# yuxng/PoseCNN

Measured on AMD Instinct MI355X. Metric: RGB-D frames/sec (640x480, 21 classes), higher is better.
Workload: dtype f32

## Files before the change

### posecnn_amd/_lib.py

```python
import ctypes
import os
from ctypes import (POINTER, c_char_p, c_float, c_int, c_int32, c_int64, c_size_t, c_uint64, c_void_p)

_HERE = os.path.dirname(os.path.abspath(__file__))
LIB_PATH = os.path.join(_HERE, "libposecnn_hip.so")

PCNN_OK = 0
PCNN_EINVAL = -1
PCNN_EWORKSPACE = -2
PCNN_EHIP = -3
PCNN_ENULL = -4

MAX_ROI = 128
HOUGH_ROWS_CAPACITY = MAX_ROI * 9
VERTEX_CHANNELS = 3
POSE_CHANNELS = 4

_P = c_void_p

SIGNATURES = {
    "pcnn_abi_version": (c_int, []),
    "pcnn_last_error_string": (c_char_p, []),
    "pcnn_status_string": (c_char_p, [c_int]),
    "pcnn_hough_voting_workspace_bytes": (c_int, [c_int, c_int, c_int, c_int, c_float, c_int, c_int, POINTER(c_size_t)]),
# ... 129 lines not shown
    "pcnn_bias_relu_train_bwd": (c_int, [_P, _P, c_int64, c_int, c_int, _P, _P, _P, c_size_t, _P]),
}

POSE3D_SIGNATURES = {
    "pcnn_pose3d_workspace_bytes": (c_int, [c_int, c_int, c_int, c_int, c_int, POINTER(c_size_t)]),
    "pcnn_pose3d_prepare_fwd": (c_int, [_P, _P, _P, _P, _P, c_float, c_int, c_int, c_int, c_int, _P, _P, _P, _P]),
    "pcnn_pose3d_sample_fwd": (c_int, [_P, _P, _P, _P, _P, _P, c_uint64, c_uint64, c_int, c_int, c_int, c_int, c_int, c_int, c_int,
                                       c_float, c_float, _P, _P, _P, _P, _P]),
    "pcnn_pose3d_round_fwd": (c_int, [_P, _P, _P, _P, _P, c_int, c_int, c_int, c_int, c_int, c_int, c_int, c_int, c_float,
                                      _P, _P, _P, _P]),
    "pcnn_pose3d_estimate_fwd": (c_int, [_P, _P, _P, _P, _P, _P, c_float, c_uint64, c_uint64, c_int, c_int, c_int, c_int,
                                         c_int, c_int, c_int, c_int, c_int, c_float, c_float, c_int,
                                         _P, _P, _P, _P, _P, _P, c_size_t, _P]),
}


def profile_enable(on=True):
    check("pcnn_profile_enable", lib().pcnn_profile_enable(1 if on else 0))


def profile_report(reset=True):
    import json
    L = lib()
    n = L.pcnn_profile_report(None, 0)
    buf = ctypes.create_string_buffer(int(n) + 16)
    L.pcnn_profile_report(buf, len(buf))
    if reset:
        L.pcnn_profile_reset()
    rep = json.loads(buf.value.decode())
    return {k.strip("()"): v for k, v in rep.items()}
# ... 8 lines not shown
        self.status = status


def lib():
    global _lib
    if _lib is None:
        if not os.path.exists(LIB_PATH):
            raise RuntimeError(
                "libposecnn_hip.so not found at %s — build it with "
                "`python -c 'import __graft_entry__ as g; g.build()'` or "
                "`make -C posecnn_amd/csrc`. There is no CPU/PyTorch fallback." % LIB_PATH)
        import torch
        handle = ctypes.CDLL(LIB_PATH)
        for name, (res, args) in list(SIGNATURES.items()) + list(TRAIN_SIGNATURES.items()) + list(FRONTEND_SIGNATURES.items()) +\
                list(SYNTH_SIGNATURES.items()) + list(AUGMENT_SIGNATURES.items()) + list(LOSS_SIGNATURES.items()) +\
                list(VERTEX_LOSS_SIGNATURES.items()) + list(TRUNK_TRAIN_SIGNATURES.items()) + list(POSE3D_SIGNATURES.items()):
            fn = getattr(handle, name)
            fn.restype = res
            fn.argtypes = args
        if handle.pcnn_abi_version() != 2:
            raise RuntimeError("libposecnn_hip.so ABI version mismatch")
        _lib = handle
    return _lib


def check(fn_name, status):
    if status != PCNN_OK:
        msg = lib().pcnn_last_error_string()
        msg = msg.decode("utf-8", "replace") if msg else ""
        if status in (PCNN_EINVAL, PCNN_ENULL):
            raise ValueError("%s: %s" % (fn_name, msg))
# ... 2 lines not shown
```

### posecnn_amd/csrc/mfma_ring.h

```cpp
#pragma once

namespace pcnn {

typedef float v4f __attribute__((ext_vector_type(4)));

__device__ __forceinline__ void glds16_s(const char* sbase, unsigned voff, unsigned lds_addr)
{
  asm volatile("s_mov_b32 m0, %2\n\tglobal_load_lds_dwordx4 %0, %1"
               :: "v"(voff), "s"(sbase), "s"(lds_addr) : "memory", "m0");
}

__device__ __forceinline__ int ring_src_col(int lr, int row) { return (lr ^ (row & 15)) * 4; }
__device__ __forceinline__ unsigned ring_chunk_bytes(int j, int lk, int lr) { return (unsigned)(((4 * j + lk) ^ lr) * 16); }

}

#define RING_DSREAD_B128(DST, ADDR, OFF) asm volatile("ds_read_b128 %0, %1 offset:%2" : "=v"(DST) : "v"(ADDR), "i"(OFF))
```

### posecnn_amd/csrc/wino_mfma.hip

```cpp
#include <cstdlib>

#include "pcnn_device.h"
#include "mfma_ring.h"

namespace {

using namespace pcnn;

constexpr int WM_BC = 64;
constexpr int WM_KC = 64;
constexpr int WM_LD = 64;
constexpr int WM_NBUF = 3;
constexpr int WM_BT = 32;
constexpr int WM_NW = 4;
constexpr int WM_UB = WM_BC / 4 / WM_NW;

enum : int {
  ABL_NO_BARRIER = 1,
  ABL_NO_DMA = 2,
  ABL_NO_LDS_READS = 4,
  ABL_NO_MFMA = 8,
  ABL_NO_FOLD = 16,
  ABL_NO_EPILOGUE = 32,
  ABL_L2_OPERANDS = 64,
  ABL_NO_STORES = 128,
  ABL_EPI_REGS_ONLY = 256,
  ABL_NT_STORES = 512,
};

template <int POOL, int ABL = 0>
__global__ __launch_bounds__(64 * WM_NW, 2) void wino43_mfma_kernel(
    const float* __restrict__ v, const float* __restrict__ ut, const float* __restrict__ bias,
    float* __restrict__ y, float* __restrict__ ypool, int H, int W, int Cin, int Cout, int Ht, int Wt,
    long long T, long long tiles_per_group, int relu, int nbt, int ncb, int ksplit, long long ysplit_stride, int mode)
{
  constexpr int RING = WM_NBUF * (WM_BT + 64) * WM_LD, STAGE2 = 2 * WM_BT * 4 * 64;
  __shared__ __attribute__((aligned(16))) float smem[RING > STAGE2 ? RING : STAGE2];

  const int x = blockIdx.x & 7, q = blockIdx.x >> 3;
  const bool cbmajor = (mode & 1) != 0;
  const int cb = cbmajor ? x : q % ncb;
  const int tb = cbmajor ? q : (q / ncb) * 8 + x;
  if (tb >= nbt) return;
  const int tb_data = (ABL & ABL_L2_OPERANDS) ? 0 : tb, cb_data = (ABL & ABL_L2_OPERANDS) ? 0 : cb;
  y += (long long)blockIdx.y * ysplit_stride;

  const int tid = threadIdx.x, lane = tid & 63;
  const int wave = __builtin_amdgcn_readfirstlane(tid >> 6);
  const int lr = lane & 15, lk = lane >> 4;
  const int nbg = (int)((tiles_per_group + WM_BT - 1) / WM_BT);
  const int grp = tb / nbg;
// ... 32 lines not shown
#pragma unroll
  for (int b = 0; b < 2; b++)
#pragma unroll
    for (int i = 0; i < 2; i++)
#pragma unroll
      for (int o = 0; o < 16; o++) yo2[b][i][o] = (v2f){0.f, 0.f};

#define WM_DMA(BUF, VO, UO)                                                  \
  if constexpr (!(ABL & ABL_NO_DMA)) {                                       \
    const char* vs_ = vbase + (VO) * 4;                                      \
    const char* us_ = ubase + (UO) * 4;                                      \
    const unsigned la_ = lds_a0 + (unsigned)(BUF) * (WM_BT * WM_LD * 4);       \
    const unsigned lb_ = lds_b0 + (unsigned)(BUF) * (64 * WM_LD * 4);          \
    glds16_s(vs_, va0, la_);                                                 \
    glds16_s(vs_, va1, la_ + 4 * WM_LD * 4);                                 \
    _Pragma("unroll") for (int i_ = 0; i_ < WM_UB; i_++)                      \
      glds16_s(us_, ub[i_], lb_ + 4 * i_ * WM_LD * 4);                        \
  }

  int pnu = 0, pxi = 0, pkc = 0;
  long long pvo = (long long)ks * NK * WM_KC, puo = pvo;
  const long long kback = (long long)(NK - 1) * WM_KC;
  const long long dvx = 6 * vplane - kback, dux = 6 * uplane - kback;
  const long long dvn = -29 * vplane - kback, dun = -29 * uplane - kback;
#define WM_PF_ADVANCE()                                                                          \
  do {                                                                                           \
    if (pkc + 1 < NK) { pkc++; pvo += WM_KC; puo += WM_KC; }                    \
    else if (pxi < 5) { pkc = 0; pxi++; pvo += dvx; puo += dux; }        \
    else if (pnu < 5) { pkc = 0; pxi = 0; pnu++; pvo += dvn; puo += dun; }        \
  } while (0)
  { WM_DMA(0, pvo, puo); WM_PF_ADVANCE(); }
  { WM_DMA(1, pvo, puo); WM_PF_ADVANCE(); }
  int cur = 0;

  const int ra0 = lr * WM_LD, rb = (16 * wave + lr) * WM_LD;

  v4f xa0[2], xa1[2], xb[2], ya0[2], ya1[2], yb[2];
  const unsigned lds0 = (unsigned)(unsigned long long)(__attribute__((address_space(3))) float*)smem;
  unsigned adA[4], adB[4];
#pragma unroll
  for (int j = 0; j < 4; j++) {
    const unsigned chb = ring_chunk_bytes(j, lk, lr);
    adA[j] = lds0 + (unsigned)ra0 * 4u + chb;
    adB[j] = lds0 + (unsigned)(WM_NBUF * WM_BT * WM_LD + rb) * 4u + chb;
  }
#define WM_DSREAD(DST, ADDR, OFF)                                                                     \
  if constexpr (!(ABL & ABL_NO_LDS_READS)) RING_DSREAD_B128(DST, ADDR, OFF);                          \
  else asm volatile("" : "+v"(DST) : "v"(ADDR))
#define WM_READ_AT(SA0, SA1, SB, G0, CUR)                                                             \
  _Pragma("unroll") for (int g_ = 0; g_ < 2; g_++) {                                                  \
    WM_DSREAD(SB[g_], adB[(G0) + g_], (CUR) * (64 * WM_LD * 4));                                      \
    WM_DSREAD(SA0[g_], adA[(G0) + g_], (CUR) * (WM_BT * WM_LD * 4));                                  \
    WM_DSREAD(SA1[g_], adA[(G0) + g_], (CUR) * (WM_BT * WM_LD * 4) + 4096);       \
  }
#define WM_READ(SA0, SA1, SB, G0)                                                                     \
  if constexpr (ABL & ABL_NO_LDS_READS) { WM_READ_AT(SA0, SA1, SB, G0, 0); }    \
  else if (cur == 0) { WM_READ_AT(SA0, SA1, SB, G0, 0); }                                             \
  else if (cur == 1) { WM_READ_AT(SA0, SA1, SB, G0, 1); }                                             \
  else { WM_READ_AT(SA0, SA1, SB, G0, 2); }
  static_assert(WM_NBUF == 3, "WM_READ dispatches over a ring of three buffers");
#define WM_MFMA1(SA0, SA1, SB, G, ACC)                                                                \
  if constexpr (ABL & ABL_NO_MFMA) { asm volatile("" :: "v"(SA0[G]), "v"(SA1[G]), "v"(SB[G])); } else \
  _Pragma("unroll") for (int i_ = 0; i_ < 4; i_++) {                                                  \
    ACC[0] = __builtin_amdgcn_mfma_f32_16x16x4f32(SA0[G][i_], SB[G][i_], ACC[0], 0, 0, 0);            \
    ACC[1] = __builtin_amdgcn_mfma_f32_16x16x4f32(SA1[G][i_], SB[G][i_], ACC[1], 0, 0, 0);            \
  }
#define WM_MFMA(SA0, SA1, SB, ACC)                                                                    \
  WM_MFMA1(SA0, SA1, SB, 0, ACC) WM_MFMA1(SA0, SA1, SB, 1, ACC)
#define WM_MFMA1_Z(SA0, SA1, SB, G, ACC)                                                              \
  if constexpr (ABL & ABL_NO_MFMA) { asm volatile("" :: "v"(SA0[G]), "v"(SA1[G]), "v"(SB[G])); } else { \
    const v4f z_ = (v4f){0.f, 0.f, 0.f, 0.f};                                                         \
    ACC[0] = __builtin_amdgcn_mfma_f32_16x16x4f32(SA0[G][0], SB[G][0], z_, 0, 0, 0);                  \
    ACC[1] = __builtin_amdgcn_mfma_f32_16x16x4f32(SA1[G][0], SB[G][0], z_, 0, 0, 0);                  \
    _Pragma("unroll") for (int i_ = 1; i_ < 4; i_++) {                                                \
// ... 19 lines not shown
        _Pragma("unroll") for (int x_ = 0; x_ < 6; x_++) m_[x_] = (v2f){acc[x_][b_][2 * h_], acc[x_][b_][2 * h_ + 1]}; \
        const v2f s_ = m_[1] + m_[2], d_ = m_[1] - m_[2], S_ = m_[3] + m_[4], D_ = m_[3] - m_[4];   \
        t_[0] = (m_[0] + s_) + S_;                                                                  \
        t_[1] = __builtin_elementwise_fma((v2f){2.f, 2.f}, D_, d_);                                 \
        t_[2] = __builtin_elementwise_fma((v2f){4.f, 4.f}, S_, s_);                                 \
        t_[3] = __builtin_elementwise_fma((v2f){8.f, 8.f}, D_, d_) + m_[5];                         \
        _Pragma("unroll") for (int a_ = 0; a_ < 4; a_++) {                                          \
          yo2[b_][h_][4 * a_ + 0] = __builtin_elementwise_fma(t_[a_], (v2f){c0, c0}, yo2[b_][h_][4 * a_ + 0]); \
          yo2[b_][h_][4 * a_ + 1] = __builtin_elementwise_fma(t_[a_], (v2f){c1, c1}, yo2[b_][h_][4 * a_ + 1]); \
          yo2[b_][h_][4 * a_ + 2] = __builtin_elementwise_fma(t_[a_], (v2f){c2, c2}, yo2[b_][h_][4 * a_ + 2]); \
          yo2[b_][h_][4 * a_ + 3] = __builtin_elementwise_fma(t_[a_], (v2f){c3, c3}, yo2[b_][h_][4 * a_ + 3]); \
        }                                                                                           \
      }                                                                                             \
  }

#define WM_STAGE(XI, XP)                                                                              \
  do {                                                                                                \
    if constexpr (ABL & ABL_NO_BARRIER) asm volatile("s_waitcnt vmcnt(4) lgkmcnt(0)" ::: "memory");   \
    else asm volatile("s_waitcnt vmcnt(6) lgkmcnt(0)\n\ts_barrier" ::: "memory");                     \
    WM_READ(xa0, xa1, xb, 0);                                                                         \
    __builtin_amdgcn_sched_barrier(0);    \
    if (kc > 0) { WM_MFMA(ya0, ya1, yb, acc[XI]); }                                                   \
    else if ((XI) > 0) { WM_MFMA(ya0, ya1, yb, acc[XP]); }                                            \
    else if (nu > 0) { WM_MFMA(ya0, ya1, yb, acc[5]); WM_FOLD(nup); }                                 \
    {                                                                                                 \
      const int nb = cur >= 1 ? cur - 1 : 2;            \
      WM_DMA(nb, pvo, puo);                                                                           \
      WM_PF_ADVANCE();                                                                                \
    }                                                                                                 \
    __builtin_amdgcn_sched_barrier(0);                                                                \
    asm volatile("s_waitcnt lgkmcnt(0)" ::: "memory");           \
    __builtin_amdgcn_sched_barrier(0);                                                                \
    if (kc == 0) { WM_MFMA1_Z(xa0, xa1, xb, 0, acc[XI]); }           \
    else { WM_MFMA1(xa0, xa1, xb, 0, acc[XI]); }                                                      \
    __builtin_amdgcn_sched_barrier(0);    \
    WM_READ(ya0, ya1, yb, 2);                                                                         \
    __builtin_amdgcn_sched_barrier(0);                                                                \
    WM_MFMA1(xa0, xa1, xb, 1, acc[XI]);                                                               \
    __builtin_amdgcn_sched_barrier(0);                                                                \
    asm volatile("s_waitcnt lgkmcnt(0)" ::: "memory");    \
    cur = cur == 2 ? 0 : cur + 1;                                                                     \
  } while (0)
  static_assert(2 + WM_UB == 6, "the stage barrier's vmcnt(6) counts the 2 + WM_UB DMA instructions a wave issues per stage");

  int nup = -1;
  for (int nu = 0; nu < 6; nu++) {
    for (int kc = 0; kc < NK; kc++) WM_STAGE(0, 5);
    for (int kc = 0; kc < NK; kc++) WM_STAGE(1, 0);
    for (int kc = 0; kc < NK; kc++) WM_STAGE(2, 1);
    for (int kc = 0; kc < NK; kc++) WM_STAGE(3, 2);
    for (int kc = 0; kc < NK; kc++) WM_STAGE(4, 3);
    for (int kc = 0; kc < NK; kc++) WM_STAGE(5, 4);
    nup = nu;
  }
  asm volatile("s_waitcnt lgkmcnt(0)" ::: "memory");
  __builtin_amdgcn_sched_barrier(0);
  WM_MFMA(ya0, ya1, yb, acc[5]);
  WM_FOLD(5);
  asm volatile("s_waitcnt vmcnt(0)" ::: "memory");
  __syncthreads();
#undef WM_STAGE
#undef WM_READ
#undef WM_READ_AT
#undef WM_DSREAD
#undef WM_MFMA
#undef WM_MFMA1
#undef WM_MFMA1_Z
#undef WM_FOLD
#undef WM_DMA
#undef WM_PF_ADVANCE

  if constexpr (ABL & ABL_EPI_REGS_ONLY) {
    const float bv_ = bv;
    float k_ = 0.f;
#pragma unroll
    for (int b = 0; b < 2; b++)
// ... 160 lines not shown
}

}

extern "C" int pcnn_winograd43_conv_workspace_bytes(int B, int H, int W, int Cin, int Cout, int groups, size_t* bytes)
{
  PCNN_REQUIRE(bytes, PCNN_ENULL, "winograd43_conv_workspace_bytes: NULL output");
  PCNN_REQUIRE(B >= 1 && H >= 1 && W >= 1 && Cin >= 64 && Cout >= 64 && groups >= 1 && B % groups == 0, PCNN_EINVAL,
               "winograd43_conv_workspace_bytes: bad shape");
  const long long tpg = (long long)B * ((H + 3) / 4) * ((W + 3) / 4) / groups;
  const int S = wino43_cin_split((long long)groups * ((tpg + WM_BT - 1) / WM_BT), Cout / WM_BC, Cin);
  *bytes = S > 1 ? sizeof(float) * ((size_t)S * B * H * W * Cout + (size_t)groups * Cout) : 0;
  return PCNN_OK;
}

extern "C" int pcnn_winograd43_conv_fwd(const float* v, const float* ut, const float* bias, int B, int H,
                                        int W, int Cin, int Cout, int groups, int relu, int pool,
                                        float* y, float* y_pool, void* workspace, size_t workspace_bytes,
                                        void* stream_)
{
  PCNN_REQUIRE(B >= 1 && H >= 1 && W >= 1, PCNN_EINVAL, "winograd43_conv: bad shape %dx%dx%d", B, H, W);
  PCNN_REQUIRE(Cin >= 64 && Cin % 64 == 0, PCNN_EINVAL, "winograd43_conv: input channels must be a multiple of 64 (got %d)", Cin);
  PCNN_REQUIRE(Cout >= 64 && Cout % 64 == 0, PCNN_EINVAL, "winograd43_conv: output channels must be a multiple of 64 (got %d)", Cout);
  PCNN_REQUIRE(pool >= 0 && pool <= 2, PCNN_EINVAL, "winograd43_conv: pool must be 0 (none), 1 (pooled only) or 2 (both)");
  PCNN_REQUIRE(!pool || (H % 2 == 0 && W % 2 == 0), PCNN_EINVAL, "winograd43_conv: pooling needs even height/width");
  PCNN_REQUIRE(groups >= 1 && B % groups == 0, PCNN_EINVAL, "winograd43_conv: batch %d is not a multiple of groups %d", B, groups);
  PCNN_REQUIRE(v && ut && bias && y && (pool != 2 || y_pool), PCNN_ENULL, "winograd43_conv: NULL pointer");
  PCNN_REQUIRE(aligned16(v) && aligned16(ut) && aligned16(bias) && aligned16(y) && (pool != 2 || aligned16(y_pool)), PCNN_EINVAL,
               "winograd43_conv: pointers (v, ut, bias, y, y_pool) must be 16-byte aligned");
  hipStream_t stream = (hipStream_t)stream_;
  const int Ht = (H + 3) / 4, Wt = (W + 3) / 4;
  const long long T = (long long)B * Ht * Wt;
  const long long tpg = T / groups;
  const int ncb = Cout / WM_BC;
  const long long nbt = (long long)groups * ((tpg + WM_BT - 1) / WM_BT);
  const long long blocks = ((nbt + 7) / 8) * 8 * ncb;
  PCNN_REQUIRE(blocks < (1ll << 31), PCNN_EINVAL, "winograd43_conv: grid too large");
  PCNN_REQUIRE(T * Cin < (1ll << 30) && (long long)Cout * Cin < (1ll << 30), PCNN_EINVAL,
               "winograd43_conv: a transform plane of %lld x %d (or %d x %d) floats exceeds the kernel's 32-bit byte offsets", T, Cin, Cout, Cin);
  int S = wino43_cin_split(nbt, ncb, Cin);
  const size_t out_elems = (size_t)B * H * W * Cout;
  if (S > 1 && !(workspace && aligned16(workspace) && workspace_bytes >= sizeof(float) * (S * out_elems + (size_t)groups * Cout))) S = 1;
  static const int env_mode = [] { const char* e = getenv("PCNN_WINO_MODE"); return e ? atoi(e) : -1; }();
  const double u_bytes = 36.0 * Cout * (double)Cin * 4.0 * groups, v_bytes = 36.0 * (double)T * Cin * 4.0;
  int mode = (ncb == 8 && u_bytes > v_bytes) ? 1 : 0;
  if (env_mode >= 0) mode = ((env_mode & 1) && ncb == 8) ? 1 : 0;
  const long long nblocks = (mode & 1) ? 8 * nbt : blocks;
#define WM_GO(P, Y, BIAS, RELU, KS, STRIDE) PCNN_LAUNCH((wino43_mfma_kernel<P>), dim3((unsigned)nblocks, KS), dim3(64 * WM_NW), 0, stream, v, ut, BIAS, Y, y_pool, \
                             H, W, Cin, Cout, Ht, Wt, T, tpg, RELU, (int)nbt, ncb, KS, (long long)(STRIDE), mode)
  if (S == 1) {
    if (pool == 0) WM_GO(0, y, bias, relu, 1, 0); else if (pool == 1) WM_GO(1, y, bias, relu, 1, 0); else WM_GO(2, y, bias, relu, 1, 0);
  } else {
    float* part = static_cast<float*>(workspace);
    WM_GO(0, part, (const float*)nullptr, 0, S, out_elems);
    const long long items = (long long)B * (pool ? (H / 2) * (W / 2) : H * W) * (Cout / 4);
    const unsigned rgrid = (unsigned)((items + 255) / 256 < 65536 ? (items + 255) / 256 : 65536);
    if (pool == 0)
      PCNN_LAUNCH(wino43_splitk_reduce_kernel<0>, dim3(rgrid), dim3(256), 0, stream, part, S, (long long)out_elems, bias, relu, y, y_pool, B, H, W, Cout, B / groups);
    else if (pool == 1)
      PCNN_LAUNCH(wino43_splitk_reduce_kernel<1>, dim3(rgrid), dim3(256), 0, stream, part, S, (long long)out_elems, bias, relu, y, y_pool, B, H, W, Cout, B / groups);
    else
      PCNN_LAUNCH(wino43_splitk_reduce_kernel<2>, dim3(rgrid), dim3(256), 0, stream, part, S, (long long)out_elems, bias, relu, y, y_pool, B, H, W, Cout, B / groups);
  }
  return check_launch("winograd43_conv_fwd");
}
```

### posecnn_amd/networks.py

```python
import math
import os

import numpy as np
import torch
import torch.nn.functional as F

from . import ops, pipeline

DEFAULT_PADDING = "SAME"


def layer(op):

    def layer_decorated(self, *args, **kwargs):
        name = kwargs.setdefault("name", self.get_unique_name(op.__name__))
        if len(self.inputs) == 0:
            raise RuntimeError("No input variables found for layer %s." % name)
        elif len(self.inputs) == 1:
            layer_input = self.inputs[0]
        else:
            layer_input = list(self.inputs)
        if op.__name__ == "conv" and isinstance(layer_input, _RawConv) and layer_input.first is not None:
            pass
        elif op.__name__ != "max_pool":
# ... 83 lines not shown
            return (self.gemm[2], self.gemm[3], self.gemm[4], self.gemm[1].shape[-2])
        if self.lazy12 is not None:
            return tuple(self.lazy12[0].first[0].shape[:3]) + (self.lazy12[2].shape[0],)
        if self.y is None and self.out is not None:
            return tuple(self.out.shape)
        return tuple(self.y.shape)


class Network(object):

    fused_train_epilogue = False

    def use_fused_train_epilogue(self, on=True):
        self.fused_train_epilogue = bool(on)
        return self

    def __init__(self, device="cuda", seed=3, init="he", trainable=True):
        self.inputs = []
        self.layers = {}
        self.vars = {}
        self.device = torch.device(device)
        self.trainable = trainable
        self.init = init
        self._gen = torch.Generator(device="cpu").manual_seed(seed)
        self.keep_prob_queue = 1.0
        self.conv_timing = None
        self.winograd_min_channels = 64
        self.winograd_tile = 4
        self._cache = {}
        self.winograd_mfma = True
# ... 26 lines not shown
            raise KeyError("Unknown layer name fed: %s" % name)
        if isinstance(out, _Lazy):
            out = self.layers[name] = out.fn()
        if isinstance(out, _RawConv):
            out = self.layers[name] = self._activate(out)
        return out

    def _activate(self, raw):
        if raw.out is None:
            if raw.wino is not None:
                m, B, H, W = raw.wino
                raw.out = ops.winograd_output(m, raw.bias, B, H, W, raw.relu, pool=False, tile=self.winograd_tile)
            elif raw.first is not None:
                raw.out = ops.conv3x3_c3(raw_frame_blob(raw.first[0]), raw.first[1], raw.bias, raw.relu)
            elif raw.gemm is not None:
                v, ut, B, H, W = raw.gemm
                raw.out = ops.winograd43_conv(v, ut, raw.bias, B, H, W, raw.relu, pool=0)
            elif raw.lazy12 is not None:
                pf, name12, w2 = raw.lazy12
                B, H, W = pf.shape[:3]
                raw.out = ops.winograd43_conv(self._first_conv_v(pf), self._winograd_filter(name12, w2, transposed=True), raw.bias,
                                              B, H, W, raw.relu, pool=0)
            else:
                raw.out = self._bias_act(raw.y, raw.bias, raw.relu)
        return raw.out

    def _conv12_fused_at(self, H, W):
        return self.fused_conv12 and self.winograd_mfma and H % 16 == 0 and W % 16 == 0

    def _first_conv_v(self, pf):
        x0 = pf.first[0]
        if _is_raw(x0):
            return ops.conv3x3_c3_winograd43_raw(x0 if x0.dtype == torch.uint8 else None, x0 if x0.dtype == torch.uint16 else None,
                                                 pf.first[1], pf.bias, pf.relu)
        return ops.conv3x3_c3_winograd43(x0, pf.first[1], pf.bias, pf.relu)

    def _winograd_filter(self, name, w, transposed=False):
        def build():
            u = ops.winograd_filter(w, self.winograd_tile)
            return u.transpose(1, 2).contiguous() if transposed else u
        return self._derived(("wino", name, transposed), (w,), build, self.winograd_tile)

    def _derived(self, slot, sources, build, extra=None):
        hit = self._cache.get(slot)
        if hit is not None and hit[2] == extra and len(hit[0]) == len(sources):
            held, versions = hit[0], hit[1]
            i = 0
            for s in sources:
                if s is not held[i] or s._version != versions[i]:
                    break
                i += 1
            else:
                return hit[3]
        value = build()
        self._cache[slot] = (tuple(sources), tuple(s._version for s in sources), extra, value)
        return value

    def _winograd43_tail(self, name, v, w, b, relu, B_, H_, W_, c_i, c_o, timing):
        if self.winograd_mfma and c_i % 64 == 0 and c_o % 64 == 0:
            ut = self._winograd_filter(name, w, transposed=True)
            if timing is not None:
                timing[1].record()
                self.conv_timing.append((name, timing[2], timing[2], timing[0], timing[1]))
            even = H_ % 2 == 0 and W_ % 2 == 0
            if name in self.defer_act and even:
                return _RawConv(None, b, relu, gemm=(v, ut, B_, H_, W_))
            if name in self.dual_pool and even:
                out = _RawConv(None, b, relu)
                out.out, out.pooled = ops.winograd43_conv(v, ut, b, B_, H_, W_, relu, pool=2)
                return out
            return ops.winograd43_conv(v, ut, b, B_, H_, W_, relu, pool=0)
        m = torch.bmm(v, self._winograd_filter(name, w))
        executed = 2.0 * m.numel() * c_i
        if timing is not None:
            timing[1].record()
        if name in self.defer_act:
            out = _RawConv(None, b, relu, wino=(m, B_, H_, W_))
        elif name in self.dual_pool and H_ % 2 == 0 and W_ % 2 == 0:
            out = _RawConv(None, b, relu, wino=(m, B_, H_, W_))
            out.dual = True
        else:
            out = ops.winograd_output(m, b, B_, H_, W_, relu, pool=False, tile=4)
        if timing is not None:
            e0, e1, extra = timing
            self.conv_timing.append((name, executed + extra, 2.0 * B_ * H_ * W_ * c_o * c_i * 9 + extra, e0, e1))
        return out
# ... 175 lines not shown
            out.out, out.pooled = _nhwc(act), _nhwc(pooled)
            return out
        return _nhwc(ops.bias_relu_train_(y, b, relu))

    @layer
    def max_pool(self, input, k_h, k_w, s_h, s_w, name, padding=DEFAULT_PADDING):
        assert padding in ("SAME", "VALID")
        if isinstance(input, _RawConv):
            if input.pooled is not None and (k_h, k_w, s_h, s_w) == (2, 2, 2, 2):
                return input.pooled
            if (input.out is None and (k_h, k_w, s_h, s_w) == (2, 2, 2, 2)
                    and input.shape[1] % 2 == 0 and input.shape[2] % 2 == 0):
                if input.first is not None:
                    return F.max_pool2d(_nchw(self._activate(input)), 2, 2).permute(0, 2, 3, 1).contiguous()
                if input.gemm is not None:
                    v, ut, B_, H_, W_ = input.gemm
                    return ops.winograd43_conv(v, ut, input.bias, B_, H_, W_, input.relu, pool=1)
                if input.lazy12 is not None:
                    pf, name12, w2 = input.lazy12
                    frag = self._derived(("conv12_frag", name12), (w2,),
                                         lambda: ops.conv12_fragment_major(self._winograd_filter(name12, w2, transposed=True)),
                                         self.winograd_tile)
                    x0, w1 = pf.first
                    if _is_raw(x0):
                        return ops.conv1_1_conv1_2_fused_raw(x0 if x0.dtype == torch.uint8 else None, x0 if x0.dtype == torch.uint16 else None,
                                                             w1, pf.bias, frag, input.bias, pf.relu, input.relu, ut2_layout=1)
                    return ops.conv1_1_conv1_2_fused(x0, w1, pf.bias, frag, input.bias, pf.relu, input.relu, groups=1, ut2_layout=1)
                if input.wino is not None and input.dual and self.winograd_tile == 4:
                    m, B_, H_, W_ = input.wino
                    input.out, pooled = ops.winograd43_output_both(m, input.bias, B_, H_, W_, input.relu)
                    return pooled
                if input.wino is not None:
# ... 360 lines not shown
            wt, bias = packed[li]
            if ci == 3:
                continue
            if li == 1 and self._conv12_fused_at(H, W) and pool == "pool1" and co == 64:
                frag = self._derived(("conv12_frag", "grouped"), (va[li][0], vb[li][0]), lambda: ops.conv12_fragment_major(wt))
                y = (ops.conv1_1_conv1_2_fused_raw(d, dp, packed[0][0], packed[0][1], frag, bias, ut2_layout=1) if raw
                     else ops.conv1_1_conv1_2_fused(x, packed[0][0], packed[0][1], frag, bias, groups=2, ut2_layout=1))
                h, w_ = h // 2, w_ // 2
                continue
            if li == 1:
                v = (ops.conv3x3_c3_winograd43_raw(d, dp, packed[0][0], packed[0][1], True) if raw
                     else ops.conv3x3_c3_winograd43(x, packed[0][0], packed[0][1], True, groups=2))
            else:
                v = ops.winograd_input(y, 4)
            mode = 0 if pool is None else (2 if name == "conv4_3" else 1)
            out = ops.winograd43_conv(v, wt, bias, B2, h, w_, True, pool=mode, groups=2)
            if mode == 2:
                full, y = out
            else:
                full = y = out
            if name in ("conv4_3", "conv5_3"):
                self.layers[name], self.layers[name + "_p"] = full[:B], full[B:]
            if pool is not None:
                h, w_ = h // 2, w_ // 2
                if pool == "pool4":
                    self.layers["pool4"], self.layers["pool4_p"] = y[:B], y[B:]
        return self

    def hbm_table(self, B, H, W):
        towers = 2 if self.input_format == 'RGBD' else 1
        act = lambda div, ch: 4.0 * B * (H // div) * (W // div) * ch
# ... 259 lines not shown
```

### posecnn_amd/ops.py

```python
import ctypes
from ctypes import c_size_t

import numpy as np

import torch

from . import _lib
from ._lib import HOUGH_ROWS_CAPACITY, MAX_ROI, POSE_CHANNELS, VERTEX_CHANNELS, check, lib

__all__ = [
    "hough_voting_gpu", "hough_voting_gpu_padded", "roi_pool", "roi_pool_add2", "hard_label", "conv1_1_conv1_2_fused",
    "conv1_1_conv1_2_fused_raw",
    "average_distance_loss", "backproject", "softmax_argmax", "deconv_bilinear", "bias_act_",
    "hough_voting_grad", "hard_label_grad", "hough_rows_capacity",
    "upscore_softmax_argmax", "Workspace", "vertex_targets", "smooth_l1_loss_vertex_gt",
    "depth_normals", "bilateral_filter_u8", "normal_image", "bilateral_tables", "augment_frames",
    "label_head_loss", "label_head_loss_grad", "vertex_head_loss", "vertex_head_loss_grad",
    "bias_relu_train_", "bias_relu_train_grad", "bias_relu_pool2_train", "bias_relu_pool2_train_grad",
    "estimate_poses_3d", "pose3d_prepare", "pose3d_sample", "pose3d_round",
]

INLIER_THRESHOLD = 0.9
LABEL_THRESHOLD = 500

# ... 462 lines not shown


def winograd43_output_both(m, bias, B, H, W, relu=True):
    m = _dev(m, "m", torch.float32)
    bias = _dev(bias, "bias", torch.float32)
    C = m.shape[2]
    if m.shape[0] != 36 or m.shape[1] != _wino_tiles(B, H, W, 4) or bias.numel() != C:
        raise ValueError("m must be [36, tiles, C] and bias [C]")
    y = torch.empty((B, H, W, C), dtype=torch.float32, device=m.device)
    yp = torch.empty((B, H // 2, W // 2, C), dtype=torch.float32, device=m.device)
    check("pcnn_winograd43_output_both_fwd",
          lib().pcnn_winograd43_output_both_fwd(_ptr(m), _ptr(bias), B, H, W, C, 1 if relu else 0, _ptr(y), _ptr(yp), _stream(m)))
    return y, yp


def winograd43_conv(v, ut, bias, B, H, W, relu=True, pool=0, groups=1):
    v = _dev(v, "v", torch.float32)
    ut = _dev(ut, "ut", torch.float32)
    bias = _aligned16(_dev(bias, "bias", torch.float32))
    Cin = v.shape[2]
    if ut.dim() == 3:
        ut = ut.unsqueeze(0)
    Cout = ut.shape[2]
    if (v.shape[0] != 36 or v.shape[1] != _wino_tiles(B, H, W, 4) or tuple(ut.shape) != (groups, 36, Cout, Cin)
            or bias.numel() != groups * Cout):
        raise ValueError("v must be [36, tiles, Cin], ut [groups, 36, Cout, Cin], bias [groups, Cout]")
    pool = int(pool)
    y = torch.empty((B, H // 2, W // 2, Cout) if pool == 1 else (B, H, W, Cout), dtype=torch.float32, device=v.device)
    yp = torch.empty((B, H // 2, W // 2, Cout), dtype=torch.float32, device=v.device) if pool == 2 else None
    nbytes = ctypes.c_size_t()
    check("pcnn_winograd43_conv_workspace_bytes",
          lib().pcnn_winograd43_conv_workspace_bytes(B, H, W, Cin, Cout, int(groups), ctypes.byref(nbytes)))
    ws = _ws(v.device, "wino43_conv").get(nbytes.value, v.device) if nbytes.value else None
    check("pcnn_winograd43_conv_fwd",
          lib().pcnn_winograd43_conv_fwd(_ptr(v), _ptr(ut), _ptr(bias), B, H, W, Cin, Cout, int(groups), 1 if relu else 0,
                                         pool, _ptr(y), _ptr(yp), _ptr(ws), nbytes.value, _stream(v)))
    return (y, yp) if pool == 2 else y


def fc_rows(x, wt, bias, relu=True, num_rows=None, addend=None):
    x = _dev(x, "x", torch.float32)
    wt = _dev(wt, "wt", torch.float32)
    bias = _aligned16(_dev(bias, "bias", torch.float32))
    if x.dim() != 2 or wt.dim() != 2 or wt.shape[1] != x.shape[1] or bias.numel() != wt.shape[0]:
        raise ValueError("x must be [M, K], wt [N, K], bias [N]")
    M, K = x.shape
    N = wt.shape[0]
    y = torch.empty((M, N), dtype=torch.float32, device=x.device)
    nr = _dev(num_rows, "num_rows", torch.int32) if num_rows is not None else None
    ad = _dev(addend, "addend", torch.float32) if addend is not None else None
    if ad is not None and tuple(ad.shape) != (M, N):
# ... 1016 lines not shown
```

Before: 831.2.

## Pre-pack Winograd filters into MFMA lane order and load B directly to registers

Adds a filter-packing kernel that lays out the transformed Winograd weights in per-lane MFMA fragment order. A new kernel variant then loads the B operand straight from global memory into registers instead of staging it through the LDS ring. This frees LDS and removes the B-side ds_reads. The packed bank is cached per layer and enabled by default. The trade-off is a reworked stage pipeline, with its own waitcnt accounting and an odd/even K-chunk variant, which adds register pressure and relies on global-load latency being hidden.

New measurement: 843.8, median of 6. 1.5% higher.

```diff
diff --git a/include/posecnn_hip_wino_packed.h b/include/posecnn_hip_wino_packed.h
--- /dev/null
+++ b/include/posecnn_hip_wino_packed.h
@@ -0,0 +1,23 @@
+#ifndef POSECNN_HIP_WINO_PACKED_H
+#define POSECNN_HIP_WINO_PACKED_H
+
+#include <stddef.h>
+#include <stdint.h>
+
+#ifdef __cplusplus
+extern "C" {
+#endif
+
+int pcnn_winograd43_pack_filters_fwd(const float* ut, int in_channels, int out_channels, int groups, float* utp,
+                                     void* stream);
+
+int pcnn_winograd43_conv_packed_fwd(const float* v, const float* utp, const float* bias, int batch, int height,
+                                    int width, int in_channels, int out_channels, int groups, int relu,
+                                    int pool, float* y, float* y_pool, void* workspace, size_t workspace_bytes,
+                                    void* stream);
+
+#ifdef __cplusplus
+}
+#endif
+
+#endif
diff --git a/posecnn_amd/_lib.py b/posecnn_amd/_lib.py
--- a/posecnn_amd/_lib.py
+++ b/posecnn_amd/_lib.py
@@ -167,6 +167,11 @@
                                          _P, _P, _P, _P, _P, _P, c_size_t, _P]),
 }
 
+WINO_PACKED_SIGNATURES = {
+    "pcnn_winograd43_pack_filters_fwd": (c_int, [_P, c_int, c_int, c_int, _P, _P]),
+    "pcnn_winograd43_conv_packed_fwd": (c_int, [_P, _P, _P, c_int, c_int, c_int, c_int, c_int, c_int, c_int, c_int, _P, _P, _P, c_size_t, _P]),
+}
+
 
 def profile_enable(on=True):
     check("pcnn_profile_enable", lib().pcnn_profile_enable(1 if on else 0))
@@ -205,7 +210,8 @@
         handle = ctypes.CDLL(LIB_PATH)
         for name, (res, args) in list(SIGNATURES.items()) + list(TRAIN_SIGNATURES.items()) + list(FRONTEND_SIGNATURES.items()) +\
                 list(SYNTH_SIGNATURES.items()) + list(AUGMENT_SIGNATURES.items()) + list(LOSS_SIGNATURES.items()) +\
-                list(VERTEX_LOSS_SIGNATURES.items()) + list(TRUNK_TRAIN_SIGNATURES.items()) + list(POSE3D_SIGNATURES.items()):
+                list(VERTEX_LOSS_SIGNATURES.items()) + list(TRUNK_TRAIN_SIGNATURES.items()) + list(POSE3D_SIGNATURES.items()) +\
+                list(WINO_PACKED_SIGNATURES.items()):
             fn = getattr(handle, name)
             fn.restype = res
             fn.argtypes = args
diff --git a/posecnn_amd/csrc/mfma_ring.h b/posecnn_amd/csrc/mfma_ring.h
--- a/posecnn_amd/csrc/mfma_ring.h
+++ b/posecnn_amd/csrc/mfma_ring.h
@@ -16,3 +16,6 @@
 }
 
 #define RING_DSREAD_B128(DST, ADDR, OFF) asm volatile("ds_read_b128 %0, %1 offset:%2" : "=v"(DST) : "v"(ADDR), "i"(OFF))
+
+#define RING_GLOAD_B128(DST, SBASE, VOFF, OFF) \
+  asm volatile("global_load_dwordx4 %0, %1, %2 offset:%3" : "=v"(DST) : "v"(VOFF), "s"(SBASE), "i"(OFF) : "memory")
diff --git a/posecnn_amd/csrc/wino_mfma.hip b/posecnn_amd/csrc/wino_mfma.hip
--- a/posecnn_amd/csrc/wino_mfma.hip
+++ b/posecnn_amd/csrc/wino_mfma.hip
@@ -2,6 +2,7 @@
 
 #include "pcnn_device.h"
 #include "mfma_ring.h"
+#include "../../include/posecnn_hip_wino_packed.h"
 
 namespace {
 
@@ -26,15 +27,16 @@
   ABL_NO_STORES = 128,
   ABL_EPI_REGS_ONLY = 256,
   ABL_NT_STORES = 512,
+  ABL_NO_B_LOADS = 1024,
 };
 
-template <int POOL, int ABL = 0>
+template <int POOL, int BSRC = 0, int ABL = 0, int ODD = 0>
 __global__ __launch_bounds__(64 * WM_NW, 2) void wino43_mfma_kernel(
     const float* __restrict__ v, const float* __restrict__ ut, const float* __restrict__ bias,
     float* __restrict__ y, float* __restrict__ ypool, int H, int W, int Cin, int Cout, int Ht, int Wt,
     long long T, long long tiles_per_group, int relu, int nbt, int ncb, int ksplit, long long ysplit_stride, int mode)
 {
-  constexpr int RING = WM_NBUF * (WM_BT + 64) * WM_LD, STAGE2 = 2 * WM_BT * 4 * 64;
+  constexpr int RING = WM_NBUF * (WM_BT + (BSRC == 0 ? 64 : 0)) * WM_LD, STAGE2 = 2 * WM_BT * 4 * 64;
   __shared__ __attribute__((aligned(16))) float smem[RING > STAGE2 ? RING : STAGE2];
 
   const int x = blockIdx.x & 7, q = blockIdx.x >> 3;
@@ -97,23 +99,47 @@
     const unsigned lb_ = lds_b0 + (unsigned)(BUF) * (64 * WM_LD * 4);          \
     glds16_s(vs_, va0, la_);                                                 \
     glds16_s(vs_, va1, la_ + 4 * WM_LD * 4);                                 \
-    _Pragma("unroll") for (int i_ = 0; i_ < WM_UB; i_++)                      \
-      glds16_s(us_, ub[i_], lb_ + 4 * i_ * WM_LD * 4);                        \
+    if constexpr (BSRC == 0) {                                               \
+      _Pragma("unroll") for (int i_ = 0; i_ < WM_UB; i_++)                    \
+        glds16_s(us_, ub[i_], lb_ + 4 * i_ * WM_LD * 4);                      \
+    }                                                                        \
   }
 
   int pnu = 0, pxi = 0, pkc = 0;
-  long long pvo = (long long)ks * NK * WM_KC, puo = pvo;
-  const long long kback = (long long)(NK - 1) * WM_KC;
-  const long long dvx = 6 * vplane - kback, dux = 6 * uplane - kback;
-  const long long dvn = -29 * vplane - kback, dun = -29 * uplane - kback;
+  constexpr int WM_USTEP = BSRC == 0 ? WM_KC : 16 * WM_KC;
+  long long pvo = (long long)ks * NK * WM_KC;
+  long long puo = BSRC == 0 ? pvo : ((long long)(cb_data * (WM_BC / 16) + wave) * (Cin / WM_KC) + (long long)ks * NK) * WM_USTEP;
+  const long long kback = (long long)(NK - 1) * WM_KC, ukback = (long long)(NK - 1) * WM_USTEP;
+  const long long dvx = 6 * vplane - kback, dux = 6 * uplane - ukback;
+  const long long dvn = -29 * vplane - kback, dun = -29 * uplane - ukback;
 #define WM_PF_ADVANCE()                                                                          \
   do {                                                                                           \
-    if (pkc + 1 < NK) { pkc++; pvo += WM_KC; puo += WM_KC; }                    \
+    if (pkc + 1 < NK) { pkc++; pvo += WM_KC; puo += WM_USTEP; }                 \
     else if (pxi < 5) { pkc = 0; pxi++; pvo += dvx; puo += dux; }        \
     else if (pnu < 5) { pkc = 0; pxi = 0; pnu++; pvo += dvn; puo += dun; }        \
   } while (0)
-  { WM_DMA(0, pvo, puo); WM_PF_ADVANCE(); }
-  { WM_DMA(1, pvo, puo); WM_PF_ADVANCE(); }
+  v4f bq[4][2];
+  if constexpr (BSRC == 1 && (ABL & ABL_NO_B_LOADS)) {
+#pragma unroll
+    for (int i = 0; i < 4; i++) bq[i][0] = bq[i][1] = (v4f){1.f, 1.f, 1.f, 1.f};
+  }
+  const unsigned vbo = 16u * (unsigned)lane;
+  long long pub = 0;
+#define WM_BLOAD(S, UO, J0)                                                  \
+  if constexpr (!(ABL & ABL_NO_B_LOADS)) {                                   \
+    const char* us_ = ubase + (UO) * 4;                                      \
+    RING_GLOAD_B128(S[0], us_, vbo, (J0) * 1024);                            \
+    RING_GLOAD_B128(S[1], us_, vbo, (J0) * 1024 + 1024);                     \
+  }
+  if constexpr (BSRC == 0) {
+    { WM_DMA(0, pvo, puo); WM_PF_ADVANCE(); }
+    { WM_DMA(1, pvo, puo); WM_PF_ADVANCE(); }
+  } else {
+    WM_BLOAD(bq[0], puo, 0);
+    WM_BLOAD(bq[1], puo, 2);
+    { WM_DMA(0, pvo, puo); WM_PF_ADVANCE(); }
+    { WM_DMA(1, pvo, puo); pub = puo; WM_PF_ADVANCE(); }
+  }
   int cur = 0;
 
   const int ra0 = lr * WM_LD, rb = (16 * wave + lr) * WM_LD;
@@ -141,6 +167,16 @@
   else if (cur == 0) { WM_READ_AT(SA0, SA1, SB, G0, 0); }                                             \
   else if (cur == 1) { WM_READ_AT(SA0, SA1, SB, G0, 1); }                                             \
   else { WM_READ_AT(SA0, SA1, SB, G0, 2); }
+#define WM_READA_AT(SA0, SA1, G0, CUR)                                                                \
+  _Pragma("unroll") for (int g_ = 0; g_ < 2; g_++) {                                                  \
+    WM_DSREAD(SA0[g_], adA[(G0) + g_], (CUR) * (WM_BT * WM_LD * 4));                                  \
+    WM_DSREAD(SA1[g_], adA[(G0) + g_], (CUR) * (WM_BT * WM_LD * 4) + 4096);                           \
+  }
+#define WM_READA(SA0, SA1, G0)                                                                        \
+  if constexpr (ABL & ABL_NO_LDS_READS) { WM_READA_AT(SA0, SA1, G0, 0); }                             \
+  else if (cur == 0) { WM_READA_AT(SA0, SA1, G0, 0); }                                                \
+  else if (cur == 1) { WM_READA_AT(SA0, SA1, G0, 1); }                                                \
+  else { WM_READA_AT(SA0, SA1, G0, 2); }
   static_assert(WM_NBUF == 3, "WM_READ dispatches over a ring of three buffers");
 #define WM_MFMA1(SA0, SA1, SB, G, ACC)                                                                \
   if constexpr (ABL & ABL_NO_MFMA) { asm volatile("" :: "v"(SA0[G]), "v"(SA1[G]), "v"(SB[G])); } else \
@@ -190,7 +226,7 @@
       }                                                                                             \
   }
 
-#define WM_STAGE(XI, XP)                                                                              \
+#define WM_STAGE0(XI, XP)                                                                             \
   do {                                                                                                \
     if constexpr (ABL & ABL_NO_BARRIER) asm volatile("s_waitcnt vmcnt(4) lgkmcnt(0)" ::: "memory");   \
     else asm volatile("s_waitcnt vmcnt(6) lgkmcnt(0)\n\ts_barrier" ::: "memory");                     \
@@ -219,23 +255,89 @@
   } while (0)
   static_assert(2 + WM_UB == 6, "the stage barrier's vmcnt(6) counts the 2 + WM_UB DMA instructions a wave issues per stage");
 
+  constexpr int WM_VM1 = WM_BT / 4 / WM_NW;
+#define WM_YMFMA_R(SB, ACC)                                                                           \
+  __builtin_amdgcn_sched_barrier(0); WM_MFMA(ya0, ya1, SB, ACC); __builtin_amdgcn_sched_barrier(0)
+#define WM_STAGE1(XI, XP, P, KC)                                                                      \
+  do {                                                                                                \
+    if constexpr (ABL & ABL_NO_BARRIER) asm volatile("s_waitcnt vmcnt(2) lgkmcnt(0)" ::: "memory");   \
+    else asm volatile("s_waitcnt vmcnt(2) lgkmcnt(0)\n\ts_barrier" ::: "memory");                     \
+    WM_READA(xa0, xa1, 0);                                                                            \
+    WM_BLOAD(bq[2 - 2 * (P)], pub, 0);                     \
+    __builtin_amdgcn_sched_barrier(0);                                                                \
+    if ((KC) > 0) { WM_YMFMA_R(bq[3 - 2 * (P)], acc[XI]); }                                           \
+    else if ((XI) > 0) { WM_YMFMA_R(bq[3 - 2 * (P)], acc[XP]); }                                      \
+    else if (nu > 0) { WM_YMFMA_R(bq[3 - 2 * (P)], acc[5]); WM_FOLD(nup); }                           \
+    __builtin_amdgcn_sched_barrier(0);                                                                \
+               \
+    WM_BLOAD(bq[3 - 2 * (P)], pub, 2);                                                                \
+    {                                                                                                 \
+      const int nb = cur >= 1 ? cur - 1 : 2;            \
+      WM_DMA(nb, pvo, puo);                                                                           \
+      pub = puo;                                                                                      \
+      WM_PF_ADVANCE();                                                                                \
+    }                                                                                                 \
+    __builtin_amdgcn_sched_barrier(0);                                                                \
+    asm volatile("s_waitcnt lgkmcnt(0)" ::: "memory");           \
+    __builtin_amdgcn_sched_barrier(0);                                                                \
+    if ((KC) == 0) { WM_MFMA1_Z(xa0, xa1, bq[2 * (P)], 0, acc[XI]); }    \
+    else { WM_MFMA1(xa0, xa1, bq[2 * (P)], 0, acc[XI]); }                                             \
+    __builtin_amdgcn_sched_barrier(0);                                                                \
+    WM_READA(ya0, ya1, 2);                                                                            \
+    __builtin_amdgcn_sched_barrier(0);                                                                \
+    WM_MFMA1(xa0, xa1, bq[2 * (P)], 1, acc[XI]);                                                      \
+    __builtin_amdgcn_sched_barrier(0);                                                                \
+    asm volatile("s_waitcnt lgkmcnt(0)" ::: "memory");                                                \
+    cur = cur == 2 ? 0 : cur + 1;                                                                     \
+  } while (0)
+  static_assert(WM_VM1 == 2, "the stage barrier's vmcnt(2) of BSRC = 1 counts the A DMA instructions a wave issues per stage");
+#define WM_PLANE_E(XI, XP) for (int kc = 0; kc < NK; kc += 2) { WM_STAGE1(XI, XP, 0, kc); WM_STAGE1(XI, XP, 1, kc + 1); }
+#define WM_PLANE_O(XI, XP, P0)                                                                        \
+  WM_STAGE1(XI, XP, P0, 0);                                                                           \
+  for (int kc = 1; kc < NK; kc += 2) { WM_STAGE1(XI, XP, 1 - (P0), kc); WM_STAGE1(XI, XP, P0, kc + 1); }
+
   int nup = -1;
-  for (int nu = 0; nu < 6; nu++) {
-    for (int kc = 0; kc < NK; kc++) WM_STAGE(0, 5);
-    for (int kc = 0; kc < NK; kc++) WM_STAGE(1, 0);
-    for (int kc = 0; kc < NK; kc++) WM_STAGE(2, 1);
-    for (int kc = 0; kc < NK; kc++) WM_STAGE(3, 2);
-    for (int kc = 0; kc < NK; kc++) WM_STAGE(4, 3);
-    for (int kc = 0; kc < NK; kc++) WM_STAGE(5, 4);
-    nup = nu;
-  }
-  asm volatile("s_waitcnt lgkmcnt(0)" ::: "memory");
-  __builtin_amdgcn_sched_barrier(0);
-  WM_MFMA(ya0, ya1, yb, acc[5]);
+  if constexpr (BSRC == 0) {
+    for (int nu = 0; nu < 6; nu++) {
+      for (int kc = 0; kc < NK; kc++) WM_STAGE0(0, 5);
+      for (int kc = 0; kc < NK; kc++) WM_STAGE0(1, 0);
+      for (int kc = 0; kc < NK; kc++) WM_STAGE0(2, 1);
+      for (int kc = 0; kc < NK; kc++) WM_STAGE0(3, 2);
+      for (int kc = 0; kc < NK; kc++) WM_STAGE0(4, 3);
+      for (int kc = 0; kc < NK; kc++) WM_STAGE0(5, 4);
+      nup = nu;
+    }
+  } else if constexpr (ODD == 0) {
+    for (int nu = 0; nu < 6; nu++) {
+      WM_PLANE_E(0, 5) WM_PLANE_E(1, 0) WM_PLANE_E(2, 1) WM_PLANE_E(3, 2) WM_PLANE_E(4, 3) WM_PLANE_E(5, 4)
+      nup = nu;
+    }
+  } else {
+    for (int nu = 0; nu < 6; nu++) {
+      WM_PLANE_O(0, 5, 0) WM_PLANE_O(1, 0, 1) WM_PLANE_O(2, 1, 0) WM_PLANE_O(3, 2, 1) WM_PLANE_O(4, 3, 0) WM_PLANE_O(5, 4, 1)
+      nup = nu;
+    }
+  }
+  if constexpr (BSRC == 0) {
+    asm volatile("s_waitcnt lgkmcnt(0)" ::: "memory");
+    __builtin_amdgcn_sched_barrier(0);
+    WM_MFMA(ya0, ya1, yb, acc[5]);
+  } else {
+    asm volatile("s_waitcnt vmcnt(2) lgkmcnt(0)" ::: "memory");
+    __builtin_amdgcn_sched_barrier(0);
+    WM_MFMA(ya0, ya1, bq[3], acc[5]);
+  }
   WM_FOLD(5);
   asm volatile("s_waitcnt vmcnt(0)" ::: "memory");
   __syncthreads();
-#undef WM_STAGE
+#undef WM_STAGE0
+#undef WM_STAGE1
+#undef WM_YMFMA_R
+#undef WM_PLANE_E
+#undef WM_PLANE_O
+#undef WM_BLOAD
+#undef WM_READA
+#undef WM_READA_AT
 #undef WM_READ
 #undef WM_READ_AT
 #undef WM_DSREAD
@@ -426,10 +528,10 @@
   return PCNN_OK;
 }
 
-extern "C" int pcnn_winograd43_conv_fwd(const float* v, const float* ut, const float* bias, int B, int H,
-                                        int W, int Cin, int Cout, int groups, int relu, int pool,
-                                        float* y, float* y_pool, void* workspace, size_t workspace_bytes,
-                                        void* stream_)
+static int wino43_conv_launch(bool packed, const float* v, const float* ut, const float* bias, int B, int H,
+                              int W, int Cin, int Cout, int groups, int relu, int pool,
+                              float* y, float* y_pool, void* workspace, size_t workspace_bytes,
+                              void* stream_)
 {
   PCNN_REQUIRE(B >= 1 && H >= 1 && W >= 1, PCNN_EINVAL, "winograd43_conv: bad shape %dx%dx%d", B, H, W);
   PCNN_REQUIRE(Cin >= 64 && Cin % 64 == 0, PCNN_EINVAL, "winograd43_conv: input channels must be a multiple of 64 (got %d)", Cin);
@@ -458,8 +560,14 @@
   int mode = (ncb == 8 && u_bytes > v_bytes) ? 1 : 0;
   if (env_mode >= 0) mode = ((env_mode & 1) && ncb == 8) ? 1 : 0;
   const long long nblocks = (mode & 1) ? 8 * nbt : blocks;
-#define WM_GO(P, Y, BIAS, RELU, KS, STRIDE) PCNN_LAUNCH((wino43_mfma_kernel<P>), dim3((unsigned)nblocks, KS), dim3(64 * WM_NW), 0, stream, v, ut, BIAS, Y, y_pool, \
+#define WM_GO_(K, Y, BIAS, RELU, KS, STRIDE) PCNN_LAUNCH(K, dim3((unsigned)nblocks, KS), dim3(64 * WM_NW), 0, stream, v, ut, BIAS, Y, y_pool, \
                              H, W, Cin, Cout, Ht, Wt, T, tpg, RELU, (int)nbt, ncb, KS, (long long)(STRIDE), mode)
+#define WM_GO(P, Y, BIAS, RELU, KS, STRIDE)                                      \
+  do {                                                                           \
+    if (packed && ((Cin / WM_KC / (KS)) & 1)) WM_GO_((wino43_mfma_kernel<P, 1, 0, 1>), Y, BIAS, RELU, KS, STRIDE); \
+    else if (packed) WM_GO_((wino43_mfma_kernel<P, 1>), Y, BIAS, RELU, KS, STRIDE);   \
+    else WM_GO_((wino43_mfma_kernel<P>), Y, BIAS, RELU, KS, STRIDE);             \
+  } while (0)
   if (S == 1) {
     if (pool == 0) WM_GO(0, y, bias, relu, 1, 0); else if (pool == 1) WM_GO(1, y, bias, relu, 1, 0); else WM_GO(2, y, bias, relu, 1, 0);
   } else {
@@ -474,5 +582,56 @@
     else
       PCNN_LAUNCH(wino43_splitk_reduce_kernel<2>, dim3(rgrid), dim3(256), 0, stream, part, S, (long long)out_elems, bias, relu, y, y_pool, B, H, W, Cout, B / groups);
   }
-  return check_launch("winograd43_conv_fwd");
-}
+  return check_launch(packed ? "winograd43_conv_packed_fwd" : "winograd43_conv_fwd");
+}
+
+extern "C" int pcnn_winograd43_conv_fwd(const float* v, const float* ut, const float* bias, int B, int H,
+                                        int W, int Cin, int Cout, int groups, int relu, int pool,
+                                        float* y, float* y_pool, void* workspace, size_t workspace_bytes,
+                                        void* stream_)
+{
+  return wino43_conv_launch(false, v, ut, bias, B, H, W, Cin, Cout, groups, relu, pool, y, y_pool, workspace, workspace_bytes, stream_);
+}
+
+extern "C" int pcnn_winograd43_conv_packed_fwd(const float* v, const float* utp, const float* bias, int B, int H,
+                                               int W, int Cin, int Cout, int groups, int relu, int pool,
+                                               float* y, float* y_pool, void* workspace, size_t workspace_bytes,
+                                               void* stream_)
+{
+  return wino43_conv_launch(true, v, utp, bias, B, H, W, Cin, Cout, groups, relu, pool, y, y_pool, workspace, workspace_bytes, stream_);
+}
+
+namespace {
+
+__global__ __launch_bounds__(256) void wino43_pack_filters_kernel(const float* __restrict__ ut, float* __restrict__ utp,
+                                                                  int Cin, int Cout, long long total4)
+{
+  const int nkc = Cin / WM_KC, n16n = Cout / 16;
+  for (long long o = (long long)blockIdx.x * 256 + threadIdx.x; o < total4; o += (long long)gridDim.x * 256) {
+    const int l = (int)(o & 63), j = (int)((o >> 6) & 3);
+    long long r = o >> 8;
+    const int kc = (int)(r % nkc); r /= nkc;
+    const int n16 = (int)(r % n16n);
+    const long long gk = r / n16n;
+    const int lr = l & 15, lk = l >> 4;
+    const long long src = (gk * Cout + 16 * n16 + lr) * Cin + 64 * kc + 16 * j + 4 * lk;
+    *reinterpret_cast<v4f*>(utp + 4 * o) = *reinterpret_cast<const v4f*>(ut + src);
+  }
+}
+
+}
+
+extern "C" int pcnn_winograd43_pack_filters_fwd(const float* ut, int Cin, int Cout, int groups, float* utp, void* stream_)
+{
+  PCNN_REQUIRE(Cin >= 64 && Cin % 64 == 0, PCNN_EINVAL, "winograd43_pack_filters: input channels must be a multiple of 64 (got %d)", Cin);
+  PCNN_REQUIRE(Cout >= 64 && Cout % 64 == 0, PCNN_EINVAL, "winograd43_pack_filters: output channels must be a multiple of 64 (got %d)", Cout);
+  PCNN_REQUIRE(groups >= 1, PCNN_EINVAL, "winograd43_pack_filters: groups must be positive (got %d)", groups);
+  PCNN_REQUIRE(ut && utp, PCNN_ENULL, "winograd43_pack_filters: NULL pointer");
+  PCNN_REQUIRE(ut != utp, PCNN_EINVAL, "winograd43_pack_filters: not an in-place permutation");
+  PCNN_REQUIRE(aligned16(ut) && aligned16(utp), PCNN_EINVAL, "winograd43_pack_filters: pointers (ut, utp) must be 16-byte aligned");
+  hipStream_t stream = (hipStream_t)stream_;
+  const long long total4 = (long long)groups * 36 * Cout * Cin / 4;
+  const unsigned grid = (unsigned)((total4 + 255) / 256 < 65536 ? (total4 + 255) / 256 : 65536);
+  PCNN_LAUNCH(wino43_pack_filters_kernel, dim3(grid), dim3(256), 0, stream, ut, utp, Cin, Cout, total4);
+  return check_launch("winograd43_pack_filters_fwd");
+}
diff --git a/posecnn_amd/networks.py b/posecnn_amd/networks.py
--- a/posecnn_amd/networks.py
+++ b/posecnn_amd/networks.py
@@ -121,6 +121,8 @@
     def use_fused_train_epilogue(self, on=True):
         self.fused_train_epilogue = bool(on)
         return self
+
+    winograd_packed = True
 
     def __init__(self, device="cuda", seed=3, init="he", trainable=True):
         self.inputs = []
@@ -177,13 +179,13 @@
             elif raw.first is not None:
                 raw.out = ops.conv3x3_c3(raw_frame_blob(raw.first[0]), raw.first[1], raw.bias, raw.relu)
             elif raw.gemm is not None:
-                v, ut, B, H, W = raw.gemm
-                raw.out = ops.winograd43_conv(v, ut, raw.bias, B, H, W, raw.relu, pool=0)
+                v, ut, B, H, W, pk = raw.gemm
+                raw.out = ops.winograd43_conv(v, ut, raw.bias, B, H, W, raw.relu, pool=0, packed=pk)
             elif raw.lazy12 is not None:
                 pf, name12, w2 = raw.lazy12
                 B, H, W = pf.shape[:3]
-                raw.out = ops.winograd43_conv(self._first_conv_v(pf), self._winograd_filter(name12, w2, transposed=True), raw.bias,
-                                              B, H, W, raw.relu, pool=0)
+                ut, pk = self._winograd_bank(name12, w2)
+                raw.out = ops.winograd43_conv(self._first_conv_v(pf), ut, raw.bias, B, H, W, raw.relu, pool=0, packed=pk)
             else:
                 raw.out = self._bias_act(raw.y, raw.bias, raw.relu)
         return raw.out
@@ -203,6 +205,13 @@
             u = ops.winograd_filter(w, self.winograd_tile)
             return u.transpose(1, 2).contiguous() if transposed else u
         return self._derived(("wino", name, transposed), (w,), build, self.winograd_tile)
+
+    def _winograd_bank(self, name, w):
+        if not self.winograd_packed:
+            return self._winograd_filter(name, w, transposed=True), False
+        return self._derived(("wino_packed", name), (w,),
+                             lambda: ops.winograd43_pack_filters(self._winograd_filter(name, w, transposed=True)),
+                             self.winograd_tile), True
 
     def _derived(self, slot, sources, build, extra=None):
         hit = self._cache.get(slot)
@@ -221,18 +230,18 @@
 
     def _winograd43_tail(self, name, v, w, b, relu, B_, H_, W_, c_i, c_o, timing):
         if self.winograd_mfma and c_i % 64 == 0 and c_o % 64 == 0:
-            ut = self._winograd_filter(name, w, transposed=True)
+            ut, pk = self._winograd_bank(name, w)
             if timing is not None:
                 timing[1].record()
                 self.conv_timing.append((name, timing[2], timing[2], timing[0], timing[1]))
             even = H_ % 2 == 0 and W_ % 2 == 0
             if name in self.defer_act and even:
-                return _RawConv(None, b, relu, gemm=(v, ut, B_, H_, W_))
+                return _RawConv(None, b, relu, gemm=(v, ut, B_, H_, W_, pk))
             if name in self.dual_pool and even:
                 out = _RawConv(None, b, relu)
-                out.out, out.pooled = ops.winograd43_conv(v, ut, b, B_, H_, W_, relu, pool=2)
+                out.out, out.pooled = ops.winograd43_conv(v, ut, b, B_, H_, W_, relu, pool=2, packed=pk)
                 return out
-            return ops.winograd43_conv(v, ut, b, B_, H_, W_, relu, pool=0)
+            return ops.winograd43_conv(v, ut, b, B_, H_, W_, relu, pool=0, packed=pk)
         m = torch.bmm(v, self._winograd_filter(name, w))
         executed = 2.0 * m.numel() * c_i
         if timing is not None:
@@ -438,8 +447,8 @@
                 if input.first is not None:
                     return F.max_pool2d(_nchw(self._activate(input)), 2, 2).permute(0, 2, 3, 1).contiguous()
                 if input.gemm is not None:
-                    v, ut, B_, H_, W_ = input.gemm
-                    return ops.winograd43_conv(v, ut, input.bias, B_, H_, W_, input.relu, pool=1)
+                    v, ut, B_, H_, W_, pk = input.gemm
+                    return ops.winograd43_conv(v, ut, input.bias, B_, H_, W_, input.relu, pool=1, packed=pk)
                 if input.lazy12 is not None:
                     pf, name12, w2 = input.lazy12
                     frag = self._derived(("conv12_frag", name12), (w2,),
@@ -830,7 +839,9 @@
             else:
                 v = ops.winograd_input(y, 4)
             mode = 0 if pool is None else (2 if name == "conv4_3" else 1)
-            out = ops.winograd43_conv(v, wt, bias, B2, h, w_, True, pool=mode, groups=2)
+            if self.winograd_packed:
+                wt = self._derived(("wino_packed", "grouped", li), (va[li][0], vb[li][0]), lambda: ops.winograd43_pack_filters(wt))
+            out = ops.winograd43_conv(v, wt, bias, B2, h, w_, True, pool=mode, groups=2, packed=self.winograd_packed)
             if mode == 2:
                 full, y = out
             else:
diff --git a/posecnn_amd/ops.py b/posecnn_amd/ops.py
--- a/posecnn_amd/ops.py
+++ b/posecnn_amd/ops.py
@@ -500,7 +500,19 @@
     return y, yp
 
 
-def winograd43_conv(v, ut, bias, B, H, W, relu=True, pool=0, groups=1):
+def winograd43_pack_filters(ut):
+    ut = _dev(ut, "ut", torch.float32)
+    if ut.dim() not in (3, 4) or ut.shape[-3] != 36:
+        raise ValueError("ut must be [groups, 36, Cout, Cin] or [36, Cout, Cin]")
+    groups = ut.shape[0] if ut.dim() == 4 else 1
+    Cout, Cin = ut.shape[-2], ut.shape[-1]
+    utp = torch.empty_like(ut)
+    check("pcnn_winograd43_pack_filters_fwd",
+          lib().pcnn_winograd43_pack_filters_fwd(_ptr(ut), Cin, Cout, int(groups), _ptr(utp), _stream(ut)))
+    return utp
+
+
+def winograd43_conv(v, ut, bias, B, H, W, relu=True, pool=0, groups=1, packed=False):
     v = _dev(v, "v", torch.float32)
     ut = _dev(ut, "ut", torch.float32)
     bias = _aligned16(_dev(bias, "bias", torch.float32))
@@ -518,9 +530,10 @@
     check("pcnn_winograd43_conv_workspace_bytes",
           lib().pcnn_winograd43_conv_workspace_bytes(B, H, W, Cin, Cout, int(groups), ctypes.byref(nbytes)))
     ws = _ws(v.device, "wino43_conv").get(nbytes.value, v.device) if nbytes.value else None
-    check("pcnn_winograd43_conv_fwd",
-          lib().pcnn_winograd43_conv_fwd(_ptr(v), _ptr(ut), _ptr(bias), B, H, W, Cin, Cout, int(groups), 1 if relu else 0,
-                                         pool, _ptr(y), _ptr(yp), _ptr(ws), nbytes.value, _stream(v)))
+    fn = "pcnn_winograd43_conv_packed_fwd" if packed else "pcnn_winograd43_conv_fwd"
+    check(fn,
+          getattr(lib(), fn)(_ptr(v), _ptr(ut), _ptr(bias), B, H, W, Cin, Cout, int(groups), 1 if relu else 0,
+                             pool, _ptr(y), _ptr(yp), _ptr(ws), nbytes.value, _stream(v)))
     return (y, yp) if pool == 2 else y
 
 
```
